# cg-tuwien/ppsurf

Hardware: AMD Instinct MI355X
Metric: occupancy query-points/sec @ res=257, 50NN (higher is better)
Workload: dtype f16x3

## Files before the change

ppsurf_amd/build.py:

```python
import concurrent.futures
import os
import subprocess
import sys

HERE = os.path.dirname(os.path.abspath(__file__))
CSRC = os.path.join(HERE, 'csrc')
LIB = os.path.join(HERE, 'libppsurf_amd.so')
SOURCES = ['pps_decode.hip', 'pps_knn.hip', 'pps_grow.hip', 'pps_mc.hip', 'pps_mesh.hip', 'pps_fkaconv.hip', 'pps_sample.hip', 'pps_train.hip', 'pps_csr.hip', 'pps_fka_train.hip', 'pps_bn_train.hip',
           'pps_attn_train.hip', 'pps_rows_train.hip', 'pps_gemm_train.hip', 'pps_optim.hip', 'pps_eval.hip', 'pps_vis.hip', 'pps_scan.hip', 'pps_cloud.hip', 'pps_simplify.hip', 'pps_transfer.hip', 'pps_trim.hip', 'pps_smooth.hip', 'pps_normals.hip', 'pps_fill.hip', 'pps_denoise.hip', 'pps_pieces.hip', 'pps_decimate.hip', 'pps_pack.cpp']
HEADERS = ['pps_common.h', 'pps_fka_common.h', 'pps_rows_train_impl.h', 'pps_head_chain_impl.h', 'pps_sweep.h', 'pps_rng.h', 'pps_cells.h', 'pps_tri.h', 'pps_faces.h', os.path.join('..', '..', 'include', 'ppsurf_amd.h'),
           os.path.join('..', '..', 'include', 'ppsurf_amd_ext.h')]
FLAGS = ['--offload-arch=gfx950', '-O3', '-std=c++17', '-ffp-contract=off', '-fPIC']


def _newer(path, deps):
    if not os.path.isfile(path):
        return True
    t = os.path.getmtime(path)
    return any(os.path.getmtime(d) > t for d in deps if os.path.isfile(d))


def build(force=False, verbose=False, variant=None, defines=()):
    hipcc = os.environ.get('HIPCC', '/opt/rocm/bin/hipcc')
    lib = LIB if not variant else os.path.join(HERE, 'libppsurf_amd_{}.so'.format(variant))
    objdir = os.path.join(CSRC, 'build' + ('_' + variant if variant else ''))
    os.makedirs(objdir, exist_ok=True)
    headers = [os.path.join(CSRC, h) for h in HEADERS]
    srcs = [s for s in SOURCES if os.path.isfile(os.path.join(CSRC, s))]
    jobs = []
    for s in srcs:
        src, obj = os.path.join(CSRC, s), os.path.join(objdir, os.path.splitext(s)[0] + '.o')
        if force or _newer(obj, [src] + headers):
            jobs.append([hipcc] + FLAGS + list(defines) + ['-c', src, '-o', obj])
    if jobs:
        def run(cmd):
            if verbose:
                print(' '.join(cmd), flush=True)
            return subprocess.run(cmd, stdout=subprocess.PIPE, stderr=subprocess.STDOUT, text=True)
        with concurrent.futures.ThreadPoolExecutor(max_workers=min(8, len(jobs))) as pool:
            for res in pool.map(run, jobs):
                if res.returncode != 0:
                    sys.stderr.write(res.stdout)
                    raise subprocess.CalledProcessError(res.returncode, res.args)
                if verbose and res.stdout.strip():
                    print(res.stdout)
    objs = [os.path.join(objdir, os.path.splitext(s)[0] + '.o') for s in srcs]
    if jobs or _newer(lib, objs):
        subprocess.check_call([hipcc, '--offload-arch=gfx950', '-shared', '-fPIC'] + objs + ['-o', lib])
    return lib


if __name__ == '__main__':
    argv = sys.argv[1:]
    variant, defines = None, [a for a in argv if a.startswith(('-D', '-f', '-m'))]
    if '--variant' in argv:
        variant = argv[argv.index('--variant') + 1]
    print(build(force='--force' in argv, verbose=True, variant=variant, defines=defines))
```

ppsurf_amd/csrc/pps_common.h:

```cpp
#pragma once
#include <hip/hip_runtime.h>
#include <stdint.h>

typedef float f32x4 __attribute__((ext_vector_type(4)));

#define PPS_WAVE 64
#define PPS_OK 0
#define PPS_ERR_ARG 1
#define PPS_ERR_LAUNCH 2

#define PPS_SG_MFMA 0x008
#define PPS_SG_DSREAD 0x100
#define PPS_SG_VALU 0x002

namespace pps {

__device__ __forceinline__ int lane_id() { return threadIdx.x & 63; }

template <int CTRL>
__device__ __forceinline__ float dpp_mov(float v) {
    return __builtin_bit_cast(float, __builtin_amdgcn_update_dpp(0, __builtin_bit_cast(int, v), CTRL, 0xf, 0xf, true));
}
__device__ __forceinline__ float row16_max(float v) {
    v = fmaxf(v, dpp_mov<0xB1>(v));
    v = fmaxf(v, dpp_mov<0x4E>(v));
    v = fmaxf(v, dpp_mov<0x141>(v));
    v = fmaxf(v, dpp_mov<0x140>(v));
    return v;
}
__device__ __forceinline__ float row16_sum(float v) {
    v += dpp_mov<0xB1>(v);
    v += dpp_mov<0x4E>(v);
    v += dpp_mov<0x141>(v);
    v += dpp_mov<0x140>(v);
    return v;
}

__device__ __forceinline__ float max_raw(float a, float b) {
    float r;
    asm("v_max_f32 %0, %1, %2" : "=v"(r) : "v"(a), "v"(b));
    return r;
}
__device__ __forceinline__ float max3_raw(float a, float b, float c) {
    float r;
    asm("v_max3_f32 %0, %1, %2, %3" : "=v"(r) : "v"(a), "v"(b), "v"(c));
    return r;
}

#define PPS_DPP4(OP, CTRL)                                                    \
    OP " %0, %0, %0 " CTRL " row_mask:0xf bank_mask:0xf bound_ctrl:1\n\t"      \
// ... 298 lines not shown
```

ppsurf_amd/csrc/pps_decode.hip:

```cpp
#include <cstdlib>
#include "pps_common.h"
#include "../../include/ppsurf_amd.h"

using namespace pps;

#define NT 256
#define NW (NT / 64)
#define WG_PER_CU (512 / NT)
#ifndef PPS_PRIO
#define PPS_PRIO 1
#endif
#ifndef PPS_PRIO_PN
#define PPS_PRIO_PN 1
#endif
#define CH4 2048

template <int CHUNK_F4_NEXT, int NTH = NT, class F>
__device__ __forceinline__ void stream_step(const f32x4* __restrict__ gnext, f32x4*& cur, f32x4*& nxt, F&& compute) {
    chunk_copy_async<CHUNK_F4_NEXT / NTH, NTH>(gnext, nxt);
    compute((const f32x4*)cur);
    stream_wait();
    __syncthreads();
    f32x4* t = cur; cur = nxt; nxt = t;
}

template <int CHUNK_F4_NEXT, int NTH = NT, class F>
__device__ __forceinline__ void stream_step_spread_at(const char* chunk, const unsigned (&voff)[CHUNK_F4_NEXT / NTH], f32x4*& cur, f32x4*& nxt, F&& compute) {
    f32x4* dst = nxt;
    compute((const f32x4*)cur, [&](int i) { if (i < CHUNK_F4_NEXT / NTH) chunk_copy_piece_at<NTH>(chunk, dst, i, voff[i]); });
    stream_wait();
    __syncthreads();
    f32x4* t = cur; cur = nxt; nxt = t;
}


__device__ __forceinline__ void lds_fill(float* dst, const float* __restrict__ src, int nfloats) {
    for (int i = threadIdx.x; i < nfloats; i += blockDim.x) dst[i] = src[i];
}

__device__ __forceinline__ float group_max(float v, int lo) {
    if (lo >= 2) v = max_raw(v, dpp_mov<0xB1>(v));
    if (lo >= 4) v = max_raw(v, dpp_mov<0x4E>(v));
    if (lo >= 8) v = max_raw(v, dpp_mov<0x141>(v));
    return v;
}
__device__ __forceinline__ float group_sum(float v, int lo) {
    if (lo >= 2) v += dpp_mov<0xB1>(v);
    if (lo >= 4) v += dpp_mov<0x4E>(v);
    if (lo >= 8) v += dpp_mov<0x141>(v);
    return v;
}

template <int N>
__device__ __forceinline__ void relu_blocks(f32x4* a) {
#pragma unroll
    for (int b = 0; b < N; ++b)
#pragma unroll
        for (int r = 0; r < 4; ++r) a[b][r] = fmaxf(a[b][r], 0.f);
}

extern __shared__ __attribute__((aligned(16))) char pps_smem[];

template <int BUF_F4, int FIRST_F4 = BUF_F4, int NTH = NT>
__device__ __forceinline__ void stream_begin(const f32x4* __restrict__ g, f32x4*& cur, f32x4*& nxt) {
    chunk_copy_async<FIRST_F4 / NTH, NTH>(g, (f32x4*)pps_smem);
    stream_wait();
    __syncthreads();
    cur = (f32x4*)pps_smem;
    nxt = cur + BUF_F4;
}

struct TileRow { int64_t i, c; bool valid; };
__device__ __forceinline__ TileRow tile_row(int tile, int wave, int n, int64_t m) {
    TileRow r;
    r.i = (int64_t)tile * (NW * 16) + wave * 16 + n;
    r.valid = r.i < m;
    r.c = r.valid ? r.i : m - 1;
    return r;
}

__device__ __forceinline__ void store_logits(const f32x4& o, const TileRow& q, int g, float* __restrict__ logits, float* __restrict__ occ) {
    if (q.valid && g == 0) {
        const float l0 = o.x, l1 = o.y;
        logits[q.i * 2] = l0;
        logits[q.i * 2 + 1] = l1;
        if (occ) {
            const float mx = fmaxf(l0, l1);
            const float e0 = __expf(l0 - mx), e1 = __expf(l1 - mx);
            occ[q.i] = (e0 - e1) / (e0 + e1);
        }
    }
}


#define RD_LDS_BYTES (2 * CH4 * 16 + 256 * 4)

__global__ __launch_bounds__(NT, 2) void rows_dense256_kernel(const float* __restrict__ in, int64_t rs, int64_t cs, int64_t m,
                                                              const float* __restrict__ wpack, const float* __restrict__ bias,
                                                              float* __restrict__ out) {
    float* bias_l = (float*)((f32x4*)pps_smem + 2 * CH4);
// ... 84 lines not shown
            stream_step<CH4>(wg + (c + 1) * CH4, cur, nxt,
                           [&](const f32x4* w) { dense_blocks<16, 2, 1>(a, &b[2 * c], w, bias4 + 8 * c, lane); });
#pragma unroll
        for (int c = 0; c < 8; ++c)
            stream_step<CH4>(wg + (c + 9) * CH4, cur, nxt,
                           [&](const f32x4* w) { dense_blocks<16, 2, 1>(b, &a[2 * c], w, bias4 + 64 + 8 * c, lane); });
#pragma unroll
        for (int c = 0; c < 2; ++c)
            stream_step<CH4>(wg + ((c + 17) % 18) * CH4, cur, nxt,
                           [&](const f32x4* w) { dense_blocks<16, 2, 0>(a, &b[2 * c], w, bias4 + 128 + 8 * c, lane); });

        __builtin_amdgcn_s_setprio(0);
        float e[16];
        {
            f32x4 m4[4], s4[4];
#pragma unroll
            for (int bb = 0; bb < 4; ++bb)
#pragma unroll
                for (int r = 0; r < 4; ++r) {
                    const float v = valid ? b[bb][r] : -INFINITY;
                    const float mx = row16_max(v);
                    const float ev = valid ? __expf(v - mx) : 0.f;
                    e[bb * 4 + r] = ev;
                    m4[bb][r] = mx;
                    s4[bb][r] = row16_sum(ev);
                }
            if (n < 4) {
                const f32x4 mm = (n == 0) ? m4[0] : (n == 1) ? m4[1] : (n == 2) ? m4[2] : m4[3];
                const f32x4 ss = (n == 0) ? s4[0] : (n == 1) ? s4[1] : (n == 2) ? s4[2] : s4[3];
                ((f32x4*)(msm + wave * 64))[4 * n + g] = mm;
                ((f32x4*)(mss + wave * 64))[4 * n + g] = ss;
            }
        }
        __syncthreads();
        {
            float mw[4], sw[4];
#pragma unroll
            for (int w2 = 0; w2 < 4; ++w2) { mw[w2] = msm[(wbase + w2) * 64 + lane]; sw[w2] = mss[(wbase + w2) * 64 + lane]; }
            const float M = fmaxf(fmaxf(mw[0], mw[1]), fmaxf(mw[2], mw[3]));
            float S = 0.f;
#pragma unroll
            for (int w2 = 0; w2 < 4; ++w2) S += sw[w2] * __expf(mw[w2] - M);
            f_l[wave * 64 + lane] = __expf(mw[wq] - M) / (64.f * S);
        }
        __syncthreads();
        float an = 0.f;
#pragma unroll
        for (int bb = 0; bb < 4; ++bb) {
            const f32x4 f4 = ((const f32x4*)(f_l + wave * 64))[4 * bb + g];
#pragma unroll
            for (int r = 0; r < 4; ++r) an += e[bb * 4 + r] * f4[r];
        }
        an += __shfl_xor(an, 16);
        an += __shfl_xor(an, 32);
#pragma unroll
        for (int bb = 0; bb < 16; ++bb) a[bb] *= an;
        rows16_sum_transposed(a, lane);
        ((f32x4*)(part + wave * 256))[4 * n + g] = a[0];
        __syncthreads();
        if (wq == 0 && qv) {
            f32x4 s = ((const f32x4*)(part + (wbase + 0) * 256))[lane];
            s += ((const f32x4*)(part + (wbase + 1) * 256))[lane];
            s += ((const f32x4*)(part + (wbase + 2) * 256))[lane];
            s += ((const f32x4*)(part + (wbase + 3) * 256))[lane];
            ((f32x4*)(pooled + qi * 256))[lane] = s;
        }
    }
}

#define IH_NT 512
#define IH_OB 2
#define IH_NW (IH_NT / 64)
#define IH_WG_PER_CU (512 / IH_NT)
#define IH_CH4 (CH4 * IH_OB / 2)
#define IH_NCH (32 / IH_OB + 4 / IH_OB)
static_assert(IH_OB == 2, "the weight pointer of the kernel's layer step wraps behind the step that fetches the last chunk: right for two output blocks per chunk only");
#define IH_LDS_BYTES (2 * IH_CH4 * 16 + (IP_W_XYZ + IP_NBIAS + IH_NW * 64 * 3 + IH_NW * 256) * 4)

__global__ __launch_bounds__(IH_NT, 2) void interp_pool_f16x3_kernel(const float* __restrict__ G, const float* __restrict__ pts,
                                                                     const float* __restrict__ query, const int64_t* __restrict__ idx,
                                                                     int64_t Q, int k, const float* __restrict__ wxyz,
                                                                     const f32x4* __restrict__ w16, const float* __restrict__ bias,
                                                                     float* __restrict__ pooled, int* __restrict__ range) {
    float amax = 0.f;
    float* xyz_l = (float*)((f32x4*)pps_smem + 2 * IH_CH4);
    float* bias_l = xyz_l + IP_W_XYZ;
    float* msm = bias_l + IP_NBIAS;
    float* mss = msm + IH_NW * 64;
    float* f_l = mss + IH_NW * 64;
    float* part = f_l + IH_NW * 64;
    const f32x4* bias4 = (const f32x4*)bias_l;
    const f32x4* wg = w16;
    const int lane = lane_id(), wave = threadIdx.x >> 6, n = lane & 15, g = lane >> 4;

    lds_fill(xyz_l, wxyz, IP_W_XYZ);
    lds_fill(bias_l, bias, IP_NBIAS);
    f32x4 *cur, *nxt;
    stream_begin<IH_CH4, IH_CH4, IH_NT>(wg, cur, nxt);
    unsigned voff[IH_CH4 / IH_NT];
    stream_lane_offsets<IH_NT>(voff);
    const char* const wfirst = (const char*)wg;
    const char* snext = wfirst + (size_t)IH_CH4 * 16;

    const int ntiles = (int)((Q + IH_NW / 4 - 1) / (IH_NW / 4));
    int first, count, stride;
    xcd_tile_range(ntiles, first, count, stride);
    const int wq = wave & 3, wbase = wave & ~3;
    for (int it = 0; it < count; ++it) {
        const int64_t qi = (int64_t)(first + it * stride) * (IH_NW / 4) + (wave >> 2);
        const bool qv = qi < Q;
        const int64_t qc = qv ? qi : Q - 1;
        const int row = wq * 16 + n;
        const bool valid = row < k;
        const int64_t i = idx[qc * k + (valid ? row : 0)];

        HiLo x[8], y[8];
        {
            f32x4 a[16];
            const f32x4* grow = (const f32x4*)(G + i * 256) + g;
#pragma unroll
            for (int bb = 0; bb < 16; ++bb) a[bb] = grow[4 * bb];
            const float coord = (g < 3) ? (query[qc * 3 + g] - pts[i * 3 + g]) : 0.f;
            xyz_blocks<16>(coord, a, xyz_l, lane);
            relu_blocks<16>(a);
#pragma unroll
            for (int kb = 0; kb < 8; ++kb) x[kb] = split_f16_r(amax, a[2 * kb], a[2 * kb + 1]);
        }
        __builtin_amdgcn_s_setprio(PPS_PRIO);
#define IH_STEP(LAST, IN, BIAS, ACTV, SINK)                                                                                           \
        {                                                                                                                             \
            stream_step_spread_at<IH_CH4, IH_NT>(snext, voff, cur, nxt, [&](const f32x4* w, auto&& piece) {                            \
                dense_blocks_f16x3_hook<8, IH_OB, ACTV>(IN, (const half8*)w, BIAS, lane, SINK,                                         \
                                                        [&](int ob, int kb) { if (ob == 0 && (kb & 1) == 0) piece(kb >> 1); }); });    \
            snext = (LAST) ? wfirst : snext + (size_t)IH_CH4 * 16;                                                                     \
            asm volatile("" : "+s"(snext));                                      \
        }
#pragma unroll
        for (int c = 0; c < 16 / IH_OB; ++c)
            IH_STEP(false, x, bias4 + 4 * IH_OB * c, 1, ([&](int p, const f32x4& o0, const f32x4& o1) { y[IH_OB / 2 * c + p] = split_f16_r(amax, o0, o1); }));
#pragma unroll
        for (int c = 0; c < 16 / IH_OB; ++c)
            IH_STEP(false, y, bias4 + 64 + 4 * IH_OB * c, 1, ([&](int p, const f32x4& o0, const f32x4& o1) { x[IH_OB / 2 * c + p] = split_f16_r(amax, o0, o1); }));
        f32x4 b[4];
#pragma unroll
        for (int c = 0; c < 4 / IH_OB; ++c)
            IH_STEP(c + 32 / IH_OB + 2 == IH_NCH, x, bias4 + 128 + 4 * IH_OB * c, 0,
                    ([&](int p, const f32x4& o0, const f32x4& o1) { b[IH_OB * c + 2 * p] = o0; b[IH_OB * c + 2 * p + 1] = o1; }));
#undef IH_STEP
        __builtin_amdgcn_s_setprio(0);
        float e[16];
        {
            f32x4 m4[4], s4[4];
#pragma unroll
            for (int bb = 0; bb < 4; ++bb) {
                float v[4], mx[4], sm[4];
#pragma unroll
                for (int r = 0; r < 4; ++r) mx[r] = v[r] = valid ? b[bb][r] : -INFINITY;
                row16_max4(mx[0], mx[1], mx[2], mx[3]);
#pragma unroll
                for (int r = 0; r < 4; ++r) {
                    const float ev = valid ? __expf(v[r] - mx[r]) : 0.f;
                    e[bb * 4 + r] = ev;
                    sm[r] = ev;
                }
                row16_sum4(sm[0], sm[1], sm[2], sm[3]);
                m4[bb] = f32x4{mx[0], mx[1], mx[2], mx[3]};
                s4[bb] = f32x4{sm[0], sm[1], sm[2], sm[3]};
            }
            if (n < 4) {
                const f32x4 mm = (n == 0) ? m4[0] : (n == 1) ? m4[1] : (n == 2) ? m4[2] : m4[3];
                const f32x4 ss = (n == 0) ? s4[0] : (n == 1) ? s4[1] : (n == 2) ? s4[2] : s4[3];
                ((f32x4*)(msm + wave * 64))[4 * n + g] = mm;
                ((f32x4*)(mss + wave * 64))[4 * n + g] = ss;
            }
        }
        __syncthreads();
        {
            float mw[4], sw[4];
#pragma unroll
            for (int w2 = 0; w2 < 4; ++w2) { mw[w2] = msm[(wbase + w2) * 64 + lane]; sw[w2] = mss[(wbase + w2) * 64 + lane]; }
            const float M = fmaxf(fmaxf(mw[0], mw[1]), fmaxf(mw[2], mw[3]));
            float S = 0.f;
#pragma unroll
            for (int w2 = 0; w2 < 4; ++w2) S += sw[w2] * __expf(mw[w2] - M);
            f_l[wave * 64 + lane] = __expf(mw[wq] - M) / (64.f * S);
        }
        __syncthreads();
        float an = 0.f;
#pragma unroll
        for (int bb = 0; bb < 4; ++bb) {
            const f32x4 f4 = ((const f32x4*)(f_l + wave * 64))[4 * bb + g];
#pragma unroll
            for (int r = 0; r < 4; ++r) an += e[bb * 4 + r] * f4[r];
        }
        an += __shfl_xor(an, 16);
        an += __shfl_xor(an, 32);
        f32x4 a[16];
#pragma unroll
        for (int kb = 0; kb < 8; ++kb) {
            join_f16(x[kb], a[2 * kb], a[2 * kb + 1]);
            a[2 * kb] *= an;
            a[2 * kb + 1] *= an;
        }
        rows16_sum_transposed(a, lane);
        ((f32x4*)(part + wave * 256))[4 * n + g] = a[0];
        __syncthreads();
        if (wq == 0 && qv) {
            f32x4 s = ((const f32x4*)(part + (wbase + 0) * 256))[lane];
            s += ((const f32x4*)(part + (wbase + 1) * 256))[lane];
            s += ((const f32x4*)(part + (wbase + 2) * 256))[lane];
            s += ((const f32x4*)(part + (wbase + 3) * 256))[lane];
            ((f32x4*)(pooled + qi * 256))[lane] = s;
        }
    }
    range_commit(amax, range);
}

#define IS_NT 256
#define IS_MAX_OUT 8
template <int CB, bool H>
__global__ __launch_bounds__(IS_NT) void interp_small_kernel(const float* __restrict__ G, const float* __restrict__ pts,
                                                             const float* __restrict__ query, const int64_t* __restrict__ idx,
                                                             int64_t Q, int k, const float* __restrict__ wpack, const float* __restrict__ w16,
                                                             const float* __restrict__ bias, const float* __restrict__ wtail, int nout,
                                                             float* __restrict__ out, int* __restrict__ guard) {
    constexpr int C = 16 * CB, NWX = 64 * CB, NW2 = 256 * CB * CB, NWQ = 1024 * CB, NB = 2 * C + 64, KB = CB / 2;
    if (!H) {
        if (gate_closed(guard)) return;
        if (guard != nullptr && blockIdx.x == 0 && threadIdx.x == 0) atomicAdd(guard + 1, 1);
    }
    float amax = 0.f;
    __shared__ __attribute__((aligned(16))) float lds[NWX + 2 * NW2 + NWQ + NB + 4 * 64 * 3 + 4 * C + IS_MAX_OUT * (C + 1)];
    float* xyz_l = lds;
    const f32x4* w2 = (const f32x4*)(lds + NWX);
    const f32x4* w3 = (const f32x4*)(lds + NWX + NW2);
    const f32x4* wq = (const f32x4*)(lds + NWX + 2 * NW2);
    float* bias_l = lds + NWX + 2 * NW2 + NWQ;
    float* msm = bias_l + NB;
    float* mss = msm + 256;
    float* f_l = mss + 256;
    float* part = f_l + 256;
    float* tail_l = part + 4 * C;
    const f32x4* bias4 = (const f32x4*)bias_l;
    const int lane = lane_id(), wave = threadIdx.x >> 6, n = lane & 15, g = lane >> 4;
    for (int i = threadIdx.x; i < NWX; i += IS_NT) lds[i] = wpack[i];
    {
        const float* dense = H ? w16 : wpack + NWX;
        for (int i = threadIdx.x; i < 2 * NW2 + NWQ; i += IS_NT) lds[NWX + i] = dense[i];
    }
    for (int i = threadIdx.x; i < NB; i += IS_NT) bias_l[i] = bias[i];
    for (int i = threadIdx.x; i < nout * (C + 1); i += IS_NT) tail_l[i] = wtail[i];
    __syncthreads();
    for (int64_t qi = blockIdx.x; qi < Q; qi += gridDim.x) {
        const int row = wave * 16 + n;
        const bool valid = row < k;
        const int64_t i = idx[qi * k + (valid ? row : 0)];
        f32x4 a[CB], h[CB], b[4];
        const f32x4* grow = (const f32x4*)(G + i * C) + g;
#pragma unroll
        for (int bb = 0; bb < CB; ++bb) a[bb] = grow[4 * bb];
        const float coord = (g < 3) ? (query[qi * 3 + g] - pts[i * 3 + g]) : 0.f;
        xyz_blocks<CB>(coord, a, xyz_l, lane);
        relu_blocks<CB>(a);
        if constexpr (H) {
            HiLo x[KB], y[KB];
#pragma unroll
            for (int kb = 0; kb < KB; ++kb) x[kb] = split_f16_r(amax, a[2 * kb], a[2 * kb + 1]);
            dense_blocks_f16x3<KB, CB, 1, false>(x, (const half8*)w2, bias4, lane,
                                                 [&](int p, const f32x4& o0, const f32x4& o1) { y[p] = split_f16_r(amax, o0, o1); });
            dense_blocks_f16x3<KB, CB, 1, false>(y, (const half8*)w3, bias4 + 4 * CB, lane, [&](int p, const f32x4& o0, const f32x4& o1) {
                x[p] = split_f16_r(amax, o0, o1);
                a[2 * p] = o0;
                a[2 * p + 1] = o1;
            });
            dense_blocks_f16x3<KB, 4, 0, false>(x, (const half8*)wq, bias4 + 8 * CB, lane,
                                                [&](int p, const f32x4& o0, const f32x4& o1) { b[2 * p] = o0; b[2 * p + 1] = o1; });
        } else {
            dense_blocks<CB, CB, 1>(a, h, w2, bias4, lane);
            dense_blocks<CB, CB, 1>(h, a, w3, bias4 + 4 * CB, lane);
            dense_blocks<CB, 4, 0>(a, b, wq, bias4 + 8 * CB, lane);
        }
        float e[16];
        {
            f32x4 m4[4], s4[4];
#pragma unroll
            for (int bb = 0; bb < 4; ++bb)
#pragma unroll
                for (int r = 0; r < 4; ++r) {
                    const float v = valid ? b[bb][r] : -INFINITY;
                    const float mx = row16_max(v);
                    const float ev = valid ? __expf(v - mx) : 0.f;
                    e[bb * 4 + r] = ev;
                    m4[bb][r] = mx;
                    s4[bb][r] = row16_sum(ev);
                }
            if (n < 4) {
                const f32x4 mm = (n == 0) ? m4[0] : (n == 1) ? m4[1] : (n == 2) ? m4[2] : m4[3];
                const f32x4 ss = (n == 0) ? s4[0] : (n == 1) ? s4[1] : (n == 2) ? s4[2] : s4[3];
                ((f32x4*)(msm + wave * 64))[4 * n + g] = mm;
                ((f32x4*)(mss + wave * 64))[4 * n + g] = ss;
            }
        }
        __syncthreads();
        {
            float mw[4], sw[4];
#pragma unroll
            for (int w2i = 0; w2i < 4; ++w2i) { mw[w2i] = msm[w2i * 64 + lane]; sw[w2i] = mss[w2i * 64 + lane]; }
            const float M = fmaxf(fmaxf(mw[0], mw[1]), fmaxf(mw[2], mw[3]));
            float S = 0.f;
#pragma unroll
            for (int w2i = 0; w2i < 4; ++w2i) S += sw[w2i] * __expf(mw[w2i] - M);
            f_l[wave * 64 + lane] = __expf(mw[wave] - M) / (64.f * S);
        }
        __syncthreads();
        float an = 0.f;
#pragma unroll
        for (int bb = 0; bb < 4; ++bb) {
            const f32x4 f4 = ((const f32x4*)(f_l + wave * 64))[4 * bb + g];
#pragma unroll
            for (int r = 0; r < 4; ++r) an += e[bb * 4 + r] * f4[r];
        }
        an += __shfl_xor(an, 16);
        an += __shfl_xor(an, 32);
#pragma unroll
        for (int bb = 0; bb < CB; ++bb) {
            f32x4 p;
#pragma unroll
            for (int r = 0; r < 4; ++r) p[r] = row16_sum(an * a[bb][r]);
            if (n == 0) ((f32x4*)(part + wave * C))[4 * bb + g] = p;
        }
        __syncthreads();
        if (threadIdx.x < nout) {
            float acc = tail_l[nout * C + threadIdx.x];
            for (int c = 0; c < C; ++c) acc += tail_l[threadIdx.x * C + c] * (part[c] + part[C + c] + part[2 * C + c] + part[3 * C + c]);
            out[qi * nout + threadIdx.x] = acc;
        }
    }
    if (H) range_commit(amax, guard);
}

#define PNT 256
#define PCH4 1024
#define PNW (PNT / 64)
#define PN_WG_PER_CU (512 / PNT)
#define PN_C2N (2048 / PCH4)
#define PN_C3N (8192 / PCH4)
#define PN_C2OB (8 / PN_C2N)
#define PN_C3OB (16 / PN_C3N)
#define PN_ROWF 260
#define PA_W_XYZ 256
#define PA_NBIAS 576
#define PN_PARK_ROWS 8
#define PA_LDS_BYTES (2 * PCH4 * 16 + (PA_W_XYZ + PA_NBIAS + PNW * PN_PARK_ROWS * PN_ROWF) * 4)

struct PatchPacking {
    int fb, lo, qg, tiles_per_query;
    bool packed;
};
__host__ __device__ inline PatchPacking patch_packing(int P, int mode = 1) {
    PatchPacking k;
    const int lo = P & 15;
    k.packed = mode != 0 && (P >= 16) && (lo == 2 || lo == 4 || lo == 8);
    k.fb = k.packed ? P / 16 : (P + 15) / 16;
    k.lo = k.packed ? lo : 0;
// ... 72 lines not shown
        const int row = t * 16 + n;
        const int rowc = row < P ? row : P - 1;
        coord[t] = (g < 3) ? qpatch[rowc * 3 + g] : 0.f;
    }
    f32x4 h0[T], h1[T];
    stn_chain_h_tiles<T>(coord, xyz_l, bias4, wg, cur, nxt, lane, amax, [&](int t, int bb, const f32x4& o0, const f32x4& o1) {
        h0[t] = o0; h1[t] = o1;
        if (t != T - 1) return;
        const f32x4 k0 = ((const f32x4*)prow)[4 * bb + g], k1 = ((const f32x4*)prow)[4 * (bb + 1) + g];
        float p[4], s[4];
#pragma unroll
        for (int r = 0; r < 4; ++r) {
            if constexpr (T == 3) {
                p[r] = max_raw(max3_raw(h0[0][r], h0[1][r], h0[2][r]), k0[r]);
                s[r] = max_raw(max3_raw(h1[0][r], h1[1][r], h1[2][r]), k1[r]);
            } else if constexpr (T == 2) {
                p[r] = max3_raw(h0[0][r], h0[1][r], k0[r]);
                s[r] = max3_raw(h1[0][r], h1[1][r], k1[r]);
            } else {
                p[r] = max_raw(h0[0][r], k0[r]);
                s[r] = max_raw(h1[0][r], k1[r]);
            }
        }
        row16_max4(p[0], p[1], p[2], p[3]);
        row16_max4(s[0], s[1], s[2], s[3]);
        if (n == 0 && store) {
            ((f32x4*)gq)[4 * bb + g] = f32x4{p[0], p[1], p[2], p[3]};
            ((f32x4*)gq)[4 * (bb + 1) + g] = f32x4{s[0], s[1], s[2], s[3]};
        }
    });
}

template <bool H>
__global__ __launch_bounds__(PNT, 2) void pointnet_stn_rows_kernel(const float* __restrict__ patches, int64_t Q, int P, int pack, int tmax,
                                                                   const float* __restrict__ wpack, const f32x4* __restrict__ wdense,
                                                                   const float* __restrict__ bias, float* __restrict__ gout, int* __restrict__ flag) {
    if (!H && gate_closed(flag)) return;
    float amax = 0.f;
    float* xyz_l = (float*)((f32x4*)pps_smem + 2 * PCH4);
    float* bias_l = xyz_l + PA_W_XYZ;
    float* park = bias_l + PA_NBIAS;
    const f32x4* bias4 = (const f32x4*)bias_l;
    const f32x4* wg = wdense;
    const int lane = lane_id(), wave = threadIdx.x >> 6, n = lane & 15, g = lane >> 4;
    float* mypark = park + wave * PN_PARK_ROWS * PN_ROWF;

    lds_fill(xyz_l, wpack, PA_W_XYZ);
    lds_fill(bias_l, bias, PA_NBIAS);
    f32x4 *cur, *nxt;
    stream_begin<PCH4, 1024, PNT>(wg, cur, nxt);

    const PatchPacking pk = patch_packing(P, pack);
    const int64_t ngroups = (Q + pk.qg - 1) / pk.qg;
    const int ntiles = (int)((ngroups + PNW - 1) / PNW);
    const bool one_pass = H && tmax >= 3 && pk.fb <= 3;
    if (one_pass && !pk.packed)
        for (int i = lane; i < PN_ROWF; i += 64) mypark[i] = -INFINITY;
    int first, count, stride;
    xcd_tile_range(ntiles, first, count, stride);
    for (int it = 0; it < count; ++it) {
        const int64_t q0 = ((int64_t)(first + it * stride) * PNW + wave) * pk.qg;
        if constexpr (H) {
            if (pk.packed) {
                const int ql = n / pk.lo;
                const int64_t qq = (q0 + ql < Q) ? q0 + ql : Q - 1;
                const float coord[1] = {(g < 3) ? patches[(qq * P + pk.fb * 16 + (n % pk.lo)) * 3 + g] : 0.f};
                stn_chain_h_tiles<1>(coord, xyz_l, bias4, wg, cur, nxt, lane, amax, [&](int, int bb, const f32x4& o0, const f32x4& o1) {
                    f32x4 m0, m1;
#pragma unroll
// ... 61 lines not shown
                    for (int r = 0; r < 4; ++r) m[r] = group_max(z[bb][r], pk.lo);
                    if ((n % pk.lo) == 0) ((f32x4*)(mypark + ql * PN_ROWF))[4 * bb + g] = m;
                }
            }
            for (int qi = 0; qi < pk.qg; ++qi) {
                const int64_t q = q0 + qi;
                const bool qv = q < Q;
                const int64_t qc = qv ? q : Q - 1;
                f32x4 rmax[16];
#pragma unroll
                for (int bb = 0; bb < 16; ++bb)
                    rmax[bb] = pk.packed ? ((const f32x4*)(mypark + qi * PN_ROWF))[4 * bb + g] : f32x4{-INFINITY, -INFINITY, -INFINITY, -INFINITY};
                for (int rb = 0; rb < pk.fb; ++rb) {
                    const int row = rb * 16 + n;
                    const int rowc = row < P ? row : P - 1;
                    const float coord = (g < 3) ? patches[(qc * P + rowc) * 3 + g] : 0.f;
                    stn_chain(coord, z, xyz_l, bias4, wg, cur, nxt, lane);
#pragma unroll
                    for (int bb = 0; bb < 16; ++bb)
#pragma unroll
                        for (int r = 0; r < 4; ++r) rmax[bb][r] = max_raw(rmax[bb][r], z[bb][r]);
                }
#pragma unroll
                for (int bb = 0; bb < 16; ++bb) {
                    float p0 = rmax[bb][0], p1 = rmax[bb][1], p2 = rmax[bb][2], p3 = rmax[bb][3];
                    row16_max4(p0, p1, p2, p3);
                    const f32x4 p = {p0, p1, p2, p3};
                    if (n == 0 && qv) ((f32x4*)(gout + q * 256))[4 * bb + g] = p;
                }
            }
        }
    }
    if (H) range_commit(amax, flag);
}

#define PB_NBIAS (128 + 64 + 4096)
#define PB_LDS_BYTES (2 * CH4 * 16 + 4096 * 4)

__global__ __launch_bounds__(NT, 2) void pointnet_stn_fc_kernel(const float* __restrict__ gin, int64_t Q,
                                                                const float* __restrict__ wpack, const float* __restrict__ bias,
                                                                float* __restrict__ trans2, const int* __restrict__ gate) {
    if (gate_closed(gate)) return;
    float* bias_l = (float*)((f32x4*)pps_smem + 2 * CH4);
    const f32x4* bias4 = (const f32x4*)bias_l;
    const f32x4* wg = (const f32x4*)wpack;
    const int lane = lane_id(), wave = threadIdx.x >> 6, n = lane & 15, g = lane >> 4;

    lds_fill(bias_l, bias + 192, 4096);
    const f32x4* bias_g = (const f32x4*)bias;
    f32x4 *cur, *nxt;
    stream_begin<CH4>(wg, cur, nxt);

    const int ntiles = (int)((Q + NW * 16 - 1) / (NW * 16));
    int first, count, stride;
    xcd_tile_range(ntiles, first, count, stride);
    for (int it = 0; it < count; ++it) {
        const TileRow q = tile_row(first + it * stride, wave, n, Q);
        f32x4 a[16], h[8], u[4];
        {
            const f32x4* src = (const f32x4*)(gin + q.c * 256) + g;
#pragma unroll
            for (int bb = 0; bb < 16; ++bb) a[bb] = src[4 * bb];
        }
#pragma unroll
        for (int c = 0; c < 4; ++c)
            stream_step<CH4>(wg + (c + 1) * CH4, cur, nxt,
// ... 136 lines not shown
            a[1] = split_f16_r(amax, x0[2], x0[3]);
            dense_blocks_f16x3<2, 8, 1>(a, (const half8*)w_c2, bias4 + 48, lane, [&](int i, const f32x4& o0, const f32x4& o1) {
                const f32x4 w0 = u4[4 * (2 * i) + g], w1 = u4[4 * (2 * i + 1) + g];
#pragma unroll
                for (int r = 0; r < 4; ++r) s += w0[r] * o0[r] + w1[r] * o1[r];
                y[2 * i] = o0;
                y[2 * i + 1] = o1;
            });
        } else {
            f32x4 x1[4];
            dense_blocks<4, 4, 1>(x0, x1, w_c0b, bias4 + 16, lane);
#pragma unroll
            for (int ob = 0; ob < 4; ++ob) {
                f32x4 o = bias4[32 + 4 * ob + g];
#pragma unroll
                for (int kb = 0; kb < 4; ++kb) {
                    o = __builtin_amdgcn_mfma_f32_16x16x4f32(tf[ob][kb].x, x1[kb].x, o, 0, 0, 0);
                    o = __builtin_amdgcn_mfma_f32_16x16x4f32(tf[ob][kb].y, x1[kb].y, o, 0, 0, 0);
                    o = __builtin_amdgcn_mfma_f32_16x16x4f32(tf[ob][kb].z, x1[kb].z, o, 0, 0, 0);
                    o = __builtin_amdgcn_mfma_f32_16x16x4f32(tf[ob][kb].w, x1[kb].w, o, 0, 0, 0);
                }
#pragma unroll
                for (int r = 0; r < 4; ++r) x0[ob][r] = fmaxf(o[r], 0.f);
            }
            dense_blocks<4, 8, 1>(x0, y, w_c2, bias4 + 48, lane);
#pragma unroll
            for (int bb = 0; bb < 8; ++bb) {
                const f32x4 w4 = u4[4 * bb + g];
#pragma unroll
                for (int r = 0; r < 4; ++r) s += w4[r] * y[bb][r];
            }
        }
        __builtin_amdgcn_s_setprio(0);
        s += __shfl_xor(s, 16);
        s += __shfl_xor(s, 32);
        s += s0;
        const float mblk = row16_max(valid ? s : -INFINITY);
        const float mnew = fmaxf(mrun, mblk);
        const float scale = __expf(mrun - mnew);
        const float en = valid ? __expf(s - mnew) : 0.f;
        mrun = mnew;
        ssum = ssum * scale + en;
#pragma unroll
        for (int bb = 0; bb < 8; ++bb)
#pragma unroll
            for (int r = 0; r < 4; ++r) acc[bb][r] = acc[bb][r] * scale + en * y[bb][r];
    }
    const float inv = 1.f / row16_sum(ssum);
    rows16_sum_transposed8(acc, lane);
    if (n < 8) ((f32x4*)(xbar + q * 128))[4 * n + g] = acc[0] * inv;
}

template <bool H>
__global__ __launch_bounds__(PNT, 2) void pointnet_feat_rows_kernel(const float* __restrict__ patches, const float* __restrict__ trans2,
                                                                    int64_t Q, int P, const float* __restrict__ wpack,
                                                                    const f32x4* __restrict__ wdense, const float* __restrict__ bias,
                                                                    float* __restrict__ xbar, int* __restrict__ flag) {
    if (!H && gate_closed(flag)) return;
    float amax = 0.f;
    const int lane = lane_id(), wave = threadIdx.x >> 6, n = lane & 15, g = lane >> 4;
    const PhaseC pc = phase_c_setup<PNT>(wpack, wdense, bias);
    __syncthreads();
    const float s0 = ((const float*)pc.bias4)[576 + 256];
    const int ntile_rows = (P + 15) / 16;

    const int ntiles = (int)((Q + PNW - 1) / PNW);
    int first, count, stride;
    xcd_tile_range(ntiles, first, count, stride);
    for (int it = 0; it < count; ++it) {
        const int64_t q = (int64_t)(first + it * stride) * PNW + wave;
        if (q >= Q) continue;
        half8 th[4][2], tl[4][2];
        f32x4 tf[4][4];
        if (H) {
            const half8* tq = (const half8*)trans2 + q * 1024 + 4 * n + g;
#pragma unroll
            for (int ob = 0; ob < 4; ++ob)
#pragma unroll
                for (int kb = 0; kb < 2; ++kb) { th[ob][kb] = tq[((ob * 2 + kb) * 2) * 64]; tl[ob][kb] = tq[((ob * 2 + kb) * 2 + 1) * 64]; }
        } else {
            const f32x4* tq = (const f32x4*)(trans2 + q * 4096);
#pragma unroll
            for (int ob = 0; ob < 4; ++ob)
#pragma unroll
                for (int kb = 0; kb < 4; ++kb) tf[ob][kb] = tq[(16 * ob + n) * 16 + 4 * kb + g];
        }
        feat_rows_query<H>(patches, q, P, ntile_rows, th, tl, tf, pc, s0, amax, lane, xbar);
    }
    if (H) range_commit(amax, flag);
}

#define PH_LDS_BYTES (2 * CH4 * 16)
__global__ __launch_bounds__(NT, 2) void pointnet_stn_head_h_kernel(const float* __restrict__ gin, int64_t Q, const f32x4* __restrict__ w16,
                                                                    const float* __restrict__ bias, half8* __restrict__ uh, int* __restrict__ range) {
    float amax = 0.f;
    const f32x4* wg = w16;
    const int lane = lane_id(), wave = threadIdx.x >> 6, n = lane & 15, g = lane >> 4;
    const f32x4* bias_g = (const f32x4*)bias;
    f32x4 *cur, *nxt;
    stream_begin<CH4>(wg, cur, nxt);
    const int ntiles = (int)((Q + NW * 16 - 1) / (NW * 16));
    int first, count, stride;
    xcd_tile_range(ntiles, first, count, stride);
    for (int it = 0; it < count; ++it) {
        const TileRow q = tile_row(first + it * stride, wave, n, Q);
        HiLo u[2];
        stn_head_h(gin + q.c * 256, wg, wg, bias_g, cur, nxt, lane, amax, u);
        if (q.valid) {
            half8* dst = uh + q.c * 16 + g;
#pragma unroll
            for (int kb = 0; kb < 2; ++kb) { dst[(2 * kb) * 4] = u[kb].hi; dst[(2 * kb + 1) * 4] = u[kb].lo; }
        }
    }
    range_commit(amax, range);
}

#define PF_NT 512
#define PF_QSTRIDE 257
#define PF_BUF (8 * PF_QSTRIDE)
#define PF_LDS_BYTES (PC_LDS_BYTES + 3 * PF_BUF * 16)
__global__ __launch_bounds__(PF_NT, 2) void pointnet_fc3_feat_rows_kernel(const float* __restrict__ patches, const half8* __restrict__ uh,
                                                                          int64_t Q, int P, const f32x4* __restrict__ wfc,
                                                                          const float* __restrict__ bias_fc, const float* __restrict__ wpack,
                                                                          const f32x4* __restrict__ wdense, const float* __restrict__ bias,
                                                                          float* __restrict__ xbar, int* __restrict__ flag) {
    float amax = 0.f;
    half8* ex = (half8*)(pps_smem + PC_LDS_BYTES);
    const int lane = lane_id(), wave = __builtin_amdgcn_readfirstlane(threadIdx.x >> 6), n = lane & 15, g = lane >> 4;
    const PhaseC pc = phase_c_setup<PF_NT>(wpack, wdense, bias);
    const float s0 = bias[576 + 256];
    const int ntile_rows = (P + 15) / 16;
    const f32x4* w3 = wfc + 5 * CH4;
    const f32x4* b3 = (const f32x4*)(bias_fc + 192);
    half8* ex_w = ex + (n < 8 ? n * PF_QSTRIDE : PF_BUF + (n - 8) * PF_QSTRIDE) + 8 * wave + g;
    const half8* ex_r = ex + wave * PF_QSTRIDE + 4 * n + g;
    const half8* ex_r2 = ex_r + PF_BUF;

    const int ntiles = (int)((Q + 15) / 16);
    int first, count, stride;
    xcd_tile_range(ntiles, first, count, stride);
    const f32x4 tf[4][4] = {};
    for (int it = 0; it < count; ++it) {
        const int64_t q0 = (int64_t)(first + it * stride) * 16;
        half8 th[4][2], tl[4][2], th2[2][2], tl2[2][2];
        {
            const int64_t qc = q0 + n < Q ? q0 + n : Q - 1;
            HiLo u[2];
#pragma unroll
            for (int kb = 0; kb < 2; ++kb) { u[kb].hi = uh[qc * 16 + (2 * kb) * 4 + g]; u[kb].lo = uh[qc * 16 + (2 * kb + 1) * 4 + g]; }
#pragma unroll
            for (int ob = 0; ob < 4; ++ob) {
                __syncthreads();
                const int c = 8 * ob + wave;
                const half8* wc = (const half8*)(w3 + c * CH4);
                asm volatile("" : "+s"(wc));
                dense_blocks_f16x3<2, 8, 0, false>(u, wc, b3 + 32 * c, lane, [&](int i, const f32x4& o0, const f32x4& o1) {
                    const HiLo v = split_f16_r(amax, o0, o1);
                    half8* d = ex_w + (n >= 8 ? (ob & 1) * PF_BUF : 0) + ((i & 1) * 2) * 64 + 4 * (i >> 1);
                    d[0] = v.hi;
                    d[64] = v.lo;
                });
                __syncthreads();
#pragma unroll
                for (int kb = 0; kb < 2; ++kb) {
                    th[ob][kb] = ex_r[(2 * kb) * 64];
                    tl[ob][kb] = ex_r[(2 * kb + 1) * 64];
                    if (ob < 2) {
                        th2[ob][kb] = ex_r2[ob * PF_BUF + (2 * kb) * 64];
                        tl2[ob][kb] = ex_r2[ob * PF_BUF + (2 * kb + 1) * 64];
                    }
                }
            }
        }
        if (q0 + wave < Q) feat_rows_query<true>(patches, q0 + wave, P, ntile_rows, th, tl, tf, pc, s0, amax, lane, xbar);
        if (q0 + wave + 8 < Q) {
#pragma unroll
            for (int kb = 0; kb < 2; ++kb) {
#pragma unroll
                for (int ob = 0; ob < 2; ++ob) {
                    th[ob][kb] = th2[ob][kb];
                    tl[ob][kb] = tl2[ob][kb];
                    th[2 + ob][kb] = ex_r2[ob * PF_BUF + (2 * kb) * 64];
                    tl[2 + ob][kb] = ex_r2[ob * PF_BUF + (2 * kb + 1) * 64];
                }
            }
            feat_rows_query<true>(patches, q0 + wave + 8, P, ntile_rows, th, tl, tf, pc, s0, amax, lane, xbar);
        }
    }
    range_commit(amax, flag);
}

#define TL_NBIAS (256 + 256 + 32)
#define TL_LDS_BYTES (2 * CH4 * 16 + TL_NBIAS * 4)

__global__ __launch_bounds__(NT, 2) void decode_tail_kernel(const float* __restrict__ pooled, const float* __restrict__ xbar, int64_t Q,
// ... 12 lines not shown

    const int ntiles = (int)((Q + NW * 16 - 1) / (NW * 16));
    int first, count, stride;
    xcd_tile_range(ntiles, first, count, stride);
    for (int it = 0; it < count; ++it) {
        const TileRow q = tile_row(first + it * stride, wave, n, Q);
        f32x4 p[16], x[8], h[16];
        {
            const f32x4* sp = (const f32x4*)(pooled + q.c * 256) + g;
            const f32x4* sx = (const f32x4*)(xbar + q.c * 128) + g;
#pragma unroll
            for (int bb = 0; bb < 16; ++bb) p[bb] = sp[4 * bb];
#pragma unroll
            for (int bb = 0; bb < 8; ++bb) x[bb] = sx[4 * bb];
        }
#pragma unroll
        for (int c = 0; c < 8; ++c)
            stream_step<CH4>(wg + (c + 1) * CH4, cur, nxt,
                           [&](const f32x4* w) { dense_blocks<16, 2, 0>(p, &h[2 * c], w, bias4 + 8 * c, lane); });
#pragma unroll
        for (int c = 0; c < 4; ++c)
            stream_step<CH4>(wg + (c + 9) * CH4, cur, nxt,
                           [&](const f32x4* w) { dense_blocks<8, 4, 1, 1>(x, &h[4 * c], w, bias4, lane); });
#pragma unroll
        for (int c = 0; c < 8; ++c)
            stream_step<CH4>(wg + (c + 13) * CH4, cur, nxt,
                           [&](const f32x4* w) { dense_blocks<16, 2, 1>(h, &p[2 * c], w, bias4 + 64 + 8 * c, lane); });
        f32x4 o[2];
        stream_step<CH4>(wg, cur, nxt, [&](const f32x4* w) { dense_blocks<16, 2, 0>(p, o, w, bias4 + 128, lane); });
        store_logits(o[0], q, g, logits, occ);
    }
}

__global__ __launch_bounds__(NT, 2) void decode_tail_h_kernel(const float* __restrict__ pooled, const float* __restrict__ xbar, int64_t Q,
                                                              const f32x4* __restrict__ w16, const float* __restrict__ bias,
                                                              float* __restrict__ logits, float* __restrict__ occ, int* __restrict__ range) {
    float amax = 0.f;
    float* bias_l = (float*)((f32x4*)pps_smem + 2 * CH4);
    const f32x4* bias4 = (const f32x4*)bias_l;
    const f32x4* wg = w16;
    const int lane = lane_id(), wave = threadIdx.x >> 6, n = lane & 15, g = lane >> 4;

    lds_fill(bias_l, bias, TL_NBIAS);
    f32x4 *cur, *nxt;
    stream_begin<CH4>(wg, cur, nxt);

    const int ntiles = (int)((Q + NW * 16 - 1) / (NW * 16));
    int first, count, stride;
    xcd_tile_range(ntiles, first, count, stride);
    for (int it = 0; it < count; ++it) {
        const TileRow q = tile_row(first + it * stride, wave, n, Q);
        HiLo p[8], x[4];
        {
            const f32x4* sp = (const f32x4*)(pooled + q.c * 256) + g;
            const f32x4* sx = (const f32x4*)(xbar + q.c * 128) + g;
#pragma unroll
            for (int kb = 0; kb < 8; ++kb) p[kb] = split_f16_r(amax, sp[4 * (2 * kb)], sp[4 * (2 * kb + 1)]);
#pragma unroll
            for (int kb = 0; kb < 4; ++kb) x[kb] = split_f16_r(amax, sx[4 * (2 * kb)], sx[4 * (2 * kb + 1)]);
        }
        HiLo y[8];
#pragma unroll
        for (int c = 0; c < 8; ++c) {
            f32x4 h[2];
            stream_step<CH4 / 2>(wg + c * 3072 + 2048, cur, nxt, [&](const f32x4* w) {
                dense_blocks_f16x3<8, 2, 0>(p, (const half8*)w, bias4 + 8 * c, lane, [&](int, const f32x4& o0, const f32x4& o1) { h[0] = o0; h[1] = o1; }); });
// ... 294 lines not shown
```

Before: 12.09 million.

## Use explicit workgroup barriers, bpermute shuffles, plain-f32 targets and wave priorities in decode

```diff
diff --git a/ppsurf_amd/build.py b/ppsurf_amd/build.py
--- a/ppsurf_amd/build.py
+++ b/ppsurf_amd/build.py
@@ -20,7 +20,7 @@
     return any(os.path.getmtime(d) > t for d in deps if os.path.isfile(d))
 
 
-def build(force=False, verbose=False, variant=None, defines=()):
+def build(force=False, verbose=False, variant=None, defines=(), only=None):
     hipcc = os.environ.get('HIPCC', '/opt/rocm/bin/hipcc')
     lib = LIB if not variant else os.path.join(HERE, 'libppsurf_amd_{}.so'.format(variant))
     objdir = os.path.join(CSRC, 'build' + ('_' + variant if variant else ''))
@@ -31,7 +31,7 @@
     for s in srcs:
         src, obj = os.path.join(CSRC, s), os.path.join(objdir, os.path.splitext(s)[0] + '.o')
         if force or _newer(obj, [src] + headers):
-            jobs.append([hipcc] + FLAGS + list(defines) + ['-c', src, '-o', obj])
+            jobs.append([hipcc] + FLAGS + (list(defines) if only in (None, s) else []) + ['-c', src, '-o', obj])
     if jobs:
         def run(cmd):
             if verbose:
@@ -52,7 +52,14 @@
 
 if __name__ == '__main__':
     argv = sys.argv[1:]
-    variant, defines = None, [a for a in argv if a.startswith(('-D', '-f', '-m'))]
+    variant, only, defines = None, None, []
+    for i, a in enumerate(argv):
+        if a == '-Xclang':
+            defines += [a, argv[i + 1]]
+        elif a.startswith(('-D', '-f', '-m')) and (i == 0 or argv[i - 1] != '-Xclang'):
+            defines.append(a)
     if '--variant' in argv:
         variant = argv[argv.index('--variant') + 1]
-    print(build(force='--force' in argv, verbose=True, variant=variant, defines=defines))
+    if '--for' in argv:
+        only = argv[argv.index('--for') + 1]
+    print(build(force='--force' in argv, verbose=True, variant=variant, defines=defines, only=only))
diff --git a/ppsurf_amd/csrc/pps_common.h b/ppsurf_amd/csrc/pps_common.h
--- a/ppsurf_amd/csrc/pps_common.h
+++ b/ppsurf_amd/csrc/pps_common.h
@@ -13,9 +13,27 @@
 #define PPS_SG_DSREAD 0x100
 #define PPS_SG_VALU 0x002
 
+#if defined(__HIP_DEVICE_COMPILE__)
+#define PPS_PLAIN_F32 __attribute__((target("no-packed-fp32-ops")))
+#else
+#define PPS_PLAIN_F32
+#endif
+
 namespace pps {
 
 __device__ __forceinline__ int lane_id() { return threadIdx.x & 63; }
+
+__device__ __forceinline__ __attribute__((convergent)) void wg_barrier() {
+    __builtin_amdgcn_fence(__ATOMIC_RELEASE, "workgroup");
+    __builtin_amdgcn_s_barrier();
+    __builtin_amdgcn_fence(__ATOMIC_ACQUIRE, "workgroup");
+}
+__device__ __forceinline__ float shfl_xor_f32(float v, int lane_mask) {
+    const int self = (int)__builtin_amdgcn_mbcnt_hi(-1, __builtin_amdgcn_mbcnt_lo(-1, 0));
+    int index = self ^ lane_mask;
+    index = index >= ((self + PPS_WAVE) & ~(PPS_WAVE - 1)) ? self : index;
+    return __builtin_bit_cast(float, __builtin_amdgcn_ds_bpermute(index << 2, __builtin_bit_cast(int, v)));
+}
 
 template <int CTRL>
 __device__ __forceinline__ float dpp_mov(float v) {
diff --git a/ppsurf_amd/csrc/pps_decode.hip b/ppsurf_amd/csrc/pps_decode.hip
--- a/ppsurf_amd/csrc/pps_decode.hip
+++ b/ppsurf_amd/csrc/pps_decode.hip
@@ -20,7 +20,7 @@
     chunk_copy_async<CHUNK_F4_NEXT / NTH, NTH>(gnext, nxt);
     compute((const f32x4*)cur);
     stream_wait();
-    __syncthreads();
+    wg_barrier();
     f32x4* t = cur; cur = nxt; nxt = t;
 }
 
@@ -29,7 +29,7 @@
     f32x4* dst = nxt;
     compute((const f32x4*)cur, [&](int i) { if (i < CHUNK_F4_NEXT / NTH) chunk_copy_piece_at<NTH>(chunk, dst, i, voff[i]); });
     stream_wait();
-    __syncthreads();
+    wg_barrier();
     f32x4* t = cur; cur = nxt; nxt = t;
 }
 
@@ -65,7 +65,7 @@
 __device__ __forceinline__ void stream_begin(const f32x4* __restrict__ g, f32x4*& cur, f32x4*& nxt) {
     chunk_copy_async<FIRST_F4 / NTH, NTH>(g, (f32x4*)pps_smem);
     stream_wait();
-    __syncthreads();
+    wg_barrier();
     cur = (f32x4*)pps_smem;
     nxt = cur + BUF_F4;
 }
@@ -216,7 +216,7 @@
                 ((f32x4*)(mss + wave * 64))[4 * n + g] = ss;
             }
         }
-        __syncthreads();
+        wg_barrier();
         {
             float mw[4], sw[4];
 #pragma unroll
@@ -227,7 +227,7 @@
             for (int w2 = 0; w2 < 4; ++w2) S += sw[w2] * __expf(mw[w2] - M);
             f_l[wave * 64 + lane] = __expf(mw[wq] - M) / (64.f * S);
         }
-        __syncthreads();
+        wg_barrier();
         float an = 0.f;
 #pragma unroll
         for (int bb = 0; bb < 4; ++bb) {
@@ -235,13 +235,13 @@
 #pragma unroll
             for (int r = 0; r < 4; ++r) an += e[bb * 4 + r] * f4[r];
         }
-        an += __shfl_xor(an, 16);
-        an += __shfl_xor(an, 32);
+        an += shfl_xor_f32(an, 16);
+        an += shfl_xor_f32(an, 32);
 #pragma unroll
         for (int bb = 0; bb < 16; ++bb) a[bb] *= an;
         rows16_sum_transposed(a, lane);
         ((f32x4*)(part + wave * 256))[4 * n + g] = a[0];
-        __syncthreads();
+        wg_barrier();
         if (wq == 0 && qv) {
             f32x4 s = ((const f32x4*)(part + (wbase + 0) * 256))[lane];
             s += ((const f32x4*)(part + (wbase + 1) * 256))[lane];
@@ -261,6 +261,7 @@
 static_assert(IH_OB == 2, "the weight pointer of the kernel's layer step wraps behind the step that fetches the last chunk: right for two output blocks per chunk only");
 #define IH_LDS_BYTES (2 * IH_CH4 * 16 + (IP_W_XYZ + IP_NBIAS + IH_NW * 64 * 3 + IH_NW * 256) * 4)
 
+PPS_PLAIN_F32
 __global__ __launch_bounds__(IH_NT, 2) void interp_pool_f16x3_kernel(const float* __restrict__ G, const float* __restrict__ pts,
                                                                      const float* __restrict__ query, const int64_t* __restrict__ idx,
                                                                      int64_t Q, int k, const float* __restrict__ wxyz,
@@ -290,6 +291,7 @@
     int first, count, stride;
     xcd_tile_range(ntiles, first, count, stride);
     const int wq = wave & 3, wbase = wave & ~3;
+    if (wave >= 4) __builtin_amdgcn_s_setprio(1);
     for (int it = 0; it < count; ++it) {
         const int64_t qi = (int64_t)(first + it * stride) * (IH_NW / 4) + (wave >> 2);
         const bool qv = qi < Q;
@@ -310,7 +312,6 @@
 #pragma unroll
             for (int kb = 0; kb < 8; ++kb) x[kb] = split_f16_r(amax, a[2 * kb], a[2 * kb + 1]);
         }
-        __builtin_amdgcn_s_setprio(PPS_PRIO);
 #define IH_STEP(LAST, IN, BIAS, ACTV, SINK)                                                                                           \
         {                                                                                                                             \
             stream_step_spread_at<IH_CH4, IH_NT>(snext, voff, cur, nxt, [&](const f32x4* w, auto&& piece) {                            \
@@ -331,7 +332,6 @@
             IH_STEP(c + 32 / IH_OB + 2 == IH_NCH, x, bias4 + 128 + 4 * IH_OB * c, 0,
                     ([&](int p, const f32x4& o0, const f32x4& o1) { b[IH_OB * c + 2 * p] = o0; b[IH_OB * c + 2 * p + 1] = o1; }));
 #undef IH_STEP
-        __builtin_amdgcn_s_setprio(0);
         float e[16];
         {
             f32x4 m4[4], s4[4];
@@ -358,7 +358,7 @@
                 ((f32x4*)(mss + wave * 64))[4 * n + g] = ss;
             }
         }
-        __syncthreads();
+        wg_barrier();
         {
             float mw[4], sw[4];
 #pragma unroll
@@ -369,7 +369,7 @@
             for (int w2 = 0; w2 < 4; ++w2) S += sw[w2] * __expf(mw[w2] - M);
             f_l[wave * 64 + lane] = __expf(mw[wq] - M) / (64.f * S);
         }
-        __syncthreads();
+        wg_barrier();
         float an = 0.f;
 #pragma unroll
         for (int bb = 0; bb < 4; ++bb) {
@@ -377,8 +377,8 @@
 #pragma unroll
             for (int r = 0; r < 4; ++r) an += e[bb * 4 + r] * f4[r];
         }
-        an += __shfl_xor(an, 16);
-        an += __shfl_xor(an, 32);
+        an += shfl_xor_f32(an, 16);
+        an += shfl_xor_f32(an, 32);
         f32x4 a[16];
 #pragma unroll
         for (int kb = 0; kb < 8; ++kb) {
@@ -388,7 +388,7 @@
         }
         rows16_sum_transposed(a, lane);
         ((f32x4*)(part + wave * 256))[4 * n + g] = a[0];
-        __syncthreads();
+        wg_barrier();
         if (wq == 0 && qv) {
             f32x4 s = ((const f32x4*)(part + (wbase + 0) * 256))[lane];
             s += ((const f32x4*)(part + (wbase + 1) * 256))[lane];
@@ -434,7 +434,7 @@
     }
     for (int i = threadIdx.x; i < NB; i += IS_NT) bias_l[i] = bias[i];
     for (int i = threadIdx.x; i < nout * (C + 1); i += IS_NT) tail_l[i] = wtail[i];
-    __syncthreads();
+    wg_barrier();
     for (int64_t qi = blockIdx.x; qi < Q; qi += gridDim.x) {
         const int row = wave * 16 + n;
         const bool valid = row < k;
@@ -485,7 +485,7 @@
                 ((f32x4*)(mss + wave * 64))[4 * n + g] = ss;
             }
         }
-        __syncthreads();
+        wg_barrier();
         {
             float mw[4], sw[4];
 #pragma unroll
@@ -496,7 +496,7 @@
             for (int w2i = 0; w2i < 4; ++w2i) S += sw[w2i] * __expf(mw[w2i] - M);
             f_l[wave * 64 + lane] = __expf(mw[wave] - M) / (64.f * S);
         }
-        __syncthreads();
+        wg_barrier();
         float an = 0.f;
 #pragma unroll
         for (int bb = 0; bb < 4; ++bb) {
@@ -504,8 +504,8 @@
 #pragma unroll
             for (int r = 0; r < 4; ++r) an += e[bb * 4 + r] * f4[r];
         }
-        an += __shfl_xor(an, 16);
-        an += __shfl_xor(an, 32);
+        an += shfl_xor_f32(an, 16);
+        an += shfl_xor_f32(an, 32);
 #pragma unroll
         for (int bb = 0; bb < CB; ++bb) {
             f32x4 p;
@@ -513,7 +513,7 @@
             for (int r = 0; r < 4; ++r) p[r] = row16_sum(an * a[bb][r]);
             if (n == 0) ((f32x4*)(part + wave * C))[4 * bb + g] = p;
         }
-        __syncthreads();
+        wg_barrier();
         if (threadIdx.x < nout) {
             float acc = tail_l[nout * C + threadIdx.x];
             for (int c = 0; c < C; ++c) acc += tail_l[threadIdx.x * C + c] * (part[c] + part[C + c] + part[2 * C + c] + part[3 * C + c]);
@@ -652,9 +652,9 @@
 }
 
 template <bool H>
-__global__ __launch_bounds__(PNT, 2) void pointnet_stn_rows_kernel(const float* __restrict__ patches, int64_t Q, int P, int pack, int tmax,
-                                                                   const float* __restrict__ wpack, const f32x4* __restrict__ wdense,
-                                                                   const float* __restrict__ bias, float* __restrict__ gout, int* __restrict__ flag) {
+__device__ __forceinline__ void pointnet_stn_rows_body(const float* __restrict__ patches, int64_t Q, int P, int pack, int tmax,
+                                                       const float* __restrict__ wpack, const f32x4* __restrict__ wdense,
+                                                       const float* __restrict__ bias, float* __restrict__ gout, int* __restrict__ flag) {
     if (!H && gate_closed(flag)) return;
     float amax = 0.f;
     float* xyz_l = (float*)((f32x4*)pps_smem + 2 * PCH4);
@@ -782,6 +782,19 @@
         }
     }
     if (H) range_commit(amax, flag);
+}
+template <bool H>
+__global__ __launch_bounds__(PNT, 2) void pointnet_stn_rows_kernel(const float* __restrict__ patches, int64_t Q, int P, int pack, int tmax,
+                                                                   const float* __restrict__ wpack, const f32x4* __restrict__ wdense,
+                                                                   const float* __restrict__ bias, float* __restrict__ gout, int* __restrict__ flag) {
+    pointnet_stn_rows_body<H>(patches, Q, P, pack, tmax, wpack, wdense, bias, gout, flag);
+}
+template <>
+PPS_PLAIN_F32
+__global__ __launch_bounds__(PNT, 2) void pointnet_stn_rows_kernel<true>(const float* __restrict__ patches, int64_t Q, int P, int pack, int tmax,
+                                                                         const float* __restrict__ wpack, const f32x4* __restrict__ wdense,
+                                                                         const float* __restrict__ bias, float* __restrict__ gout, int* __restrict__ flag) {
+    pointnet_stn_rows_body<true>(patches, Q, P, pack, tmax, wpack, wdense, bias, gout, flag);
 }
 
 #define PB_NBIAS (128 + 64 + 4096)
@@ -984,8 +997,8 @@
             }
         }
         __builtin_amdgcn_s_setprio(0);
-        s += __shfl_xor(s, 16);
-        s += __shfl_xor(s, 32);
+        s += shfl_xor_f32(s, 16);
+        s += shfl_xor_f32(s, 32);
         s += s0;
         const float mblk = row16_max(valid ? s : -INFINITY);
         const float mnew = fmaxf(mrun, mblk);
@@ -1004,15 +1017,15 @@
 }
 
 template <bool H>
-__global__ __launch_bounds__(PNT, 2) void pointnet_feat_rows_kernel(const float* __restrict__ patches, const float* __restrict__ trans2,
-                                                                    int64_t Q, int P, const float* __restrict__ wpack,
-                                                                    const f32x4* __restrict__ wdense, const float* __restrict__ bias,
-                                                                    float* __restrict__ xbar, int* __restrict__ flag) {
+__device__ __forceinline__ void pointnet_feat_rows_body(const float* __restrict__ patches, const float* __restrict__ trans2,
+                                                        int64_t Q, int P, const float* __restrict__ wpack,
+                                                        const f32x4* __restrict__ wdense, const float* __restrict__ bias,
+                                                        float* __restrict__ xbar, int* __restrict__ flag) {
     if (!H && gate_closed(flag)) return;
     float amax = 0.f;
     const int lane = lane_id(), wave = threadIdx.x >> 6, n = lane & 15, g = lane >> 4;
     const PhaseC pc = phase_c_setup<PNT>(wpack, wdense, bias);
-    __syncthreads();
+    wg_barrier();
     const float s0 = ((const float*)pc.bias4)[576 + 256];
     const int ntile_rows = (P + 15) / 16;
 
@@ -1040,6 +1053,21 @@
         feat_rows_query<H>(patches, q, P, ntile_rows, th, tl, tf, pc, s0, amax, lane, xbar);
     }
     if (H) range_commit(amax, flag);
+}
+template <bool H>
+__global__ __launch_bounds__(PNT, 2) void pointnet_feat_rows_kernel(const float* __restrict__ patches, const float* __restrict__ trans2,
+                                                                    int64_t Q, int P, const float* __restrict__ wpack,
+                                                                    const f32x4* __restrict__ wdense, const float* __restrict__ bias,
+                                                                    float* __restrict__ xbar, int* __restrict__ flag) {
+    pointnet_feat_rows_body<H>(patches, trans2, Q, P, wpack, wdense, bias, xbar, flag);
+}
+template <>
+PPS_PLAIN_F32
+__global__ __launch_bounds__(PNT, 2) void pointnet_feat_rows_kernel<true>(const float* __restrict__ patches, const float* __restrict__ trans2,
+                                                                          int64_t Q, int P, const float* __restrict__ wpack,
+                                                                          const f32x4* __restrict__ wdense, const float* __restrict__ bias,
+                                                                          float* __restrict__ xbar, int* __restrict__ flag) {
+    pointnet_feat_rows_body<true>(patches, trans2, Q, P, wpack, wdense, bias, xbar, flag);
 }
 
 #define PH_LDS_BYTES (2 * CH4 * 16)
@@ -1071,6 +1099,7 @@
 #define PF_QSTRIDE 257
 #define PF_BUF (8 * PF_QSTRIDE)
 #define PF_LDS_BYTES (PC_LDS_BYTES + 3 * PF_BUF * 16)
+PPS_PLAIN_F32
 __global__ __launch_bounds__(PF_NT, 2) void pointnet_fc3_feat_rows_kernel(const float* __restrict__ patches, const half8* __restrict__ uh,
                                                                           int64_t Q, int P, const f32x4* __restrict__ wfc,
                                                                           const float* __restrict__ bias_fc, const float* __restrict__ wpack,
@@ -1102,7 +1131,7 @@
             for (int kb = 0; kb < 2; ++kb) { u[kb].hi = uh[qc * 16 + (2 * kb) * 4 + g]; u[kb].lo = uh[qc * 16 + (2 * kb + 1) * 4 + g]; }
 #pragma unroll
             for (int ob = 0; ob < 4; ++ob) {
-                __syncthreads();
+                wg_barrier();
                 const int c = 8 * ob + wave;
                 const half8* wc = (const half8*)(w3 + c * CH4);
                 asm volatile("" : "+s"(wc));
@@ -1112,7 +1141,7 @@
                     d[0] = v.hi;
                     d[64] = v.lo;
                 });
-                __syncthreads();
+                wg_barrier();
 #pragma unroll
                 for (int kb = 0; kb < 2; ++kb) {
                     th[ob][kb] = ex_r[(2 * kb) * 64];
@@ -1191,6 +1220,7 @@
     }
 }
 
+PPS_PLAIN_F32
 __global__ __launch_bounds__(NT, 2) void decode_tail_h_kernel(const float* __restrict__ pooled, const float* __restrict__ xbar, int64_t Q,
                                                               const f32x4* __restrict__ w16, const float* __restrict__ bias,
                                                               float* __restrict__ logits, float* __restrict__ occ, int* __restrict__ range) {
```

After: 12.24 million, median of 6. 1.01x the previous value.
